# corelab-src/dacapo

Measured on AMD Instinct MI355X. Metric: NTT/s (NTT-equivalents over one run() of the ResNet HEVM program, nt=2^14), higher is better.
Workload: dtype u64; 1 GPU; ResNet-20 (SiLU) HEVM program traced from the reference's examples/benchmarks/ResNet.py with its resnet20.silu.model weights, nt=2^14 slots, N=2^15, 14 x 60-bit primes (SEAL_HEVM.cpp:39-53); one independent ciphertext stream per GPU; streams_per_gpu=1, parallelism=replicas x1 (no collective in the op path)

## Files before the change

dacapo_amd/csrc/batch_ops.hip:

```cpp
#include <stdlib.h>

#include "galois.hpp"
#include "plan.hpp"

namespace dacapo {

constexpr int kBT = 256;

__global__ __launch_bounds__(kBT) void b_tensor_kernel(const MulItem *__restrict__ items, u64 *__restrict__ target, int ell,
                                                        size_t N, const DModulus *__restrict__ mods)
{
    const int i = blockIdx.y, b = blockIdx.z;
    const MulItem it = items[b];
    const DModulus m = mods[i];
    const size_t k = ((size_t)blockIdx.x * kBT + threadIdx.x) * 2;
    const u64x2 a0 = *reinterpret_cast<const u64x2 *>(it.a.limb(0, i, N) + k), a1 = *reinterpret_cast<const u64x2 *>(it.a.limb(1, i, N) + k);
    const u64x2 b0 = *reinterpret_cast<const u64x2 *>(it.b.limb(0, i, N) + k), b1 = *reinterpret_cast<const u64x2 *>(it.b.limb(1, i, N) + k);
    u64x2 c0, c1, c2;
#pragma unroll
    for (int e = 0; e < 2; e++) {
        c0[e] = mulmod(a0[e], b0[e], m);
        Acc128 acc;
        acc.clear();
        acc.mac(a0[e], b1[e]);
// ... 95 lines not shown
        f_dr_lift_fcols(c, acc_last, acc_ps, w.tmp, 2 * B, ell, sp, s);
    } else
        f_dr_icols_lift_fcols(c, acc_last, acc_ps, w.tmp, 2 * B, ell, sp, s);
    last(fused_mac);
}
template <int MODE>
static void b_ks_tail(Context &c, const BatchWs &w, u64 *digits, const KsItem *items, const void *final_items, const u64 *shared_key, int B,
                      int ell, hipStream_t s, const Handoff &h)
{
    b_ks_tail<MODE>(c, w, digits, items, final_items, shared_key, B, ell, s, nullptr, [&](bool fused_mac) {
        f_frows_final(c, (MODE == 1 && fused_mac) ? 4 : MODE, w.tmp, final_items, w.acc, 2 * B, ell, c.K - 1, s, RsItem{}, nullptr, nullptr, h,
                      MODE == 0 && fused_mac);
    });
}

void b_rotate_hops(Context &c, const BatchWs &w, const KsItem *d_items, int B, int ell, hipStream_t s, const Handoff &h, int unique)
{
    if (c.hybrid()) {
        hyb_rotate_hops(c, w, d_items, B, ell, s, unique);
        return;
    }
    f_irows_rot_c1(c, d_items, ell, w.digits, B, s);
    b_ks_tail<0>(c, w, w.digits, d_items, d_items, nullptr, B, ell, s, h);
}

void b_mul_relin(Context &c, const BatchWs &w, const MulItem *d_items, const u64 *relin_key, int B, int ell, hipStream_t s, const Handoff &h)
{
    if (c.hybrid()) {
        hyb_mul_relin(c, w, d_items, relin_key, B, ell, s);
        return;
    }
    const size_t N = c.N;
// ... 419 lines not shown
```

dacapo_amd/csrc/c_api.hip:

```cpp
#include "../../include/dacapo_ckks.h"

#include <stddef.h>
#include <string.h>

#include <algorithm>
#include <vector>

#include "kernels.hpp"
#include "noise_stats.hpp"
#include "plan.hpp"

using namespace dacapo;

#include "c_api_types.hpp"

static inline hipStream_t S(void *s) { return (hipStream_t)s; }
static inline CtView V(const uint64_t *p, long stride) { return CtView{ const_cast<u64 *>(p), stride }; }

namespace {
constexpr int kItemSlots = 64;
constexpr size_t kItemBytes = 128;
static_assert(sizeof(KsItem) <= kItemBytes && sizeof(MulItem) <= kItemBytes && sizeof(RsItem) <= kItemBytes && sizeof(MulRsItem) <= kItemBytes, "item slot too small");
constexpr int kConstSlotWords = 64;
void *item_slot(dc_context *ctx, const void *host_item, size_t bytes, hipStream_t s)
// ... 319 lines not shown
    DC_HIP_CHECK(hipStreamSynchronize(s));
    const char *d = static_cast<const char *>(ctx->mulsum_table);
    b_mul_sum_relin(c, batch_ws(c.ws0), reinterpret_cast<const MulSumItem *>(d), reinterpret_cast<const MulTerm *>(d + kTermsAt), relin_key, 1, ell, s);
    if (alias) launch_ew(c, EwOp::Copy, V(dst, dst_stride), out, out, 2, 2, ell, s);
}
void dc_ct_rotate_hop(dc_context *ctx, uint64_t *dst, long dst_stride, const uint64_t *src, long src_stride,
                      uint32_t galois_elt, const uint64_t *galois_key, int ell, void *stream)
{
    if (overlaps(dst, src)) {
        rotate_hop(*ctx->c, ctx->c->ws0, V(dst, dst_stride), V(src, src_stride), galois_elt, galois_key, ell, S(stream));
        return;
    }
    const KsItem it{ V(src, src_stride), V(dst, dst_stride), galois_key, galois_elt, 0 };
    const KsItem *d = static_cast<const KsItem *>(item_slot(ctx, &it, sizeof(it), S(stream)));
    b_rotate_hops(*ctx->c, batch_ws(ctx->c->ws0), d, 1, ell, S(stream));
}
void dc_ct_rotate_hoisted(dc_context *ctx, uint64_t *const *dsts, long dst_stride, const uint64_t *src, long src_stride,
                          const uint32_t *galois_elts, const uint64_t *const *galois_keys, int count, int ell, void *stream)
{
    const size_t B = (size_t)count;
    const KsItem *d = hoist_items(ctx, "dc_ct_rotate_hoisted", ", where dc_ct_rotate_hop already takes the digits before the automorphism", "hops",
                                  count, ell, B, S(stream), [&](std::vector<KsItem> &h) {
                                      for (size_t b = 0; b < B; b++)
                                          h.push_back(KsItem{ V(src, src_stride), V(dsts[b], dst_stride), galois_keys[b], galois_elts[b], 0 });
                                      h.push_back(KsItem{ V(src, src_stride), V(src, src_stride), nullptr, 1u, 0 });
                                      return (size_t)0;
                                  });
    Context &c = *ctx->c;
    const BatchWs w{ c.ws0.ct_tmp, c.ws0.ks_digits, c.ws0.ks_ext, ctx->hoist_acc, ctx->hoist_tmp };
    hoist_rotate_hops(c, w, d, d + B, count, 1, ell, S(stream));
// ... 124 lines not shown
```

dacapo_amd/csrc/fused_ks.hip:

```cpp
#include "ks_mac.hpp"

namespace dacapo {

struct SrcStrided {
    const u64 *base;
    long stride;
    int prime_base, period;
    __device__ int prime(int z) const { return prime_base + z % period; }
    __device__ u64 load(int z, int g, int) const { return base[(long)z * stride + g]; }
};
template <int E>
__device__ __forceinline__ void rs_operand(u64 (&v)[E], const int (&g)[E], const RsItem &it, const SumSrc *__restrict__ srcs, int p, int i,
                                           size_t N, const DModulus &M)
{
    if (it.count == 0) {
        const u64 *x = it.src.limb(p, i, N);
#pragma unroll
        for (int j = 0; j < E; j++) v[j] = x[g[j]];
    } else {
        u64 s[E];
        Acc128 a[E];
#pragma unroll
        for (int j = 0; j < E; j++) s[j] = 0, a[j].clear();
        int n_plain = 0, n_prod = 0;
// ... 813 lines not shown
    const size_t N = (size_t)1 << logN;
    const DModulus M = mods[pm];
    const u64 *key = MODE == 0 ? items[b].key : shared_key;
    int g[E];
#pragma unroll
    for (int e = 0; e < E; e++) g[e] = tile_gidx<K, LOGE, false>(NP - 1, logN, blockIdx.x, e);
    Acc128 a0[E], a1[E];
#pragma unroll
    for (int e = 0; e < E; e++) a0[e].clear(), a1[e].clear();
    if (MODE == 0 && pmod && m < ell) {
        const KsItem &it = items[b];
        const u64 *c0 = it.src.limb(0, m, N);
        const u64 P = pmod[m];
        u64 cv[E];
        galois_gather<E>(cv, c0, (u32)g[0], it.elt, logN);
#pragma unroll
        for (int e = 0; e < E; e++) a0[e].lo = mulmod(cv[e], P, M);
    }
    if (FOLD && m == ell - 1) {
        const MulRsItem &it = reinterpret_cast<const MulRsItem *>(items)[b];
        const u64 *pa0 = it.a.limb(0, m, N), *pa1 = it.a.limb(1, m, N), *pb0 = it.b.limb(0, m, N), *pb1 = it.b.limb(1, m, N);
        const u64 *pl = it.add ? it.add + (size_t)m * N : nullptr;
        const u64 P = pmod[m];
#pragma unroll
        for (int e = 0; e < E; e++) {
            const u64 va0 = pa0[g[e]], va1 = pa1[g[e]], vb0 = pb0[g[e]], vb1 = pb1[g[e]];
            u64 d0 = mulmod(va0, vb0, M);
            if (pl) d0 = addmod(d0, pl[g[e]], M.q);
            Acc128 t;
            t.clear();
            t.mac(va0, vb1);
            t.mac(va1, vb0);
// ... 430 lines not shown
```

dacapo_amd/csrc/hevm_vm.hip:

```cpp
#include "hevm_vm.hpp"

#include "../../include/dacapo_ckks.h"
#include "c_api_types.hpp"
#include "chacha.hpp"
#include "seal_serial.hpp"

#include <math.h>
#include <string.h>
#include <sys/random.h>

#include <algorithm>
#include <cmath>
#include <chrono>
#include <fstream>
#include <iostream>

namespace dacapo {

constexpr int kVmThreads = 256;

constexpr int kRngCoefs = 8;

__device__ __forceinline__ int rng_cbd(u64 w)
{
// ... 410 lines not shown
                            "switching uses grouped digits, whose lazy sums take no addend\n", ks_flatten, ksp, alpha);
            abort();
        }
        if (!ks_hoist || !ks_lazy) {
            fprintf(stderr, "[dacapo_amd] option ks_flatten_sums = %d needs%s%s%s: a flattened stage is a hoisted lazy sum -- the rotations of one source "
                            "share its decomposition (ks_hoist) and one division by P (ks_lazy_sum)\n", ks_flatten, ks_hoist ? "" : " ks_hoist = 1",
                    !ks_hoist && !ks_lazy ? " and" : "", ks_lazy ? "" : " ks_lazy_sum >= 1");
            abort();
        }
        if (option(OPT_ROT_COMPOSE) != 0) {
            fprintf(stderr, "[dacapo_amd] option ks_flatten_sums = %d does not combine with rot_compose = 1: a memoised hop may serve two rotate "
                            "instructions, and a flattened stage takes its rotations' hops away\n", ks_flatten);
            abort();
        }
    }
    zenc_head = option(OPT_ZENC_HEAD) != 0;
    const int bits = (int)option(OPT_PRIME_BITS);
    ctx.reset(new Context(logN, K, bits, primes, ksp, alpha));
    ctx->ensure_scratch();
    encoder.reset(new HostEncoder(logN));
    use_plan = option(OPT_PLAN) != 0;
    plan_graph = option(OPT_PLAN_GRAPH) != 0;
    plan_dag = option(OPT_PLAN_GRAPH) == 2;
    plan_lanes = option(OPT_PLAN_LANES) >= 2 ? 2 : 1;
    host_encoder = option(OPT_HOST_ENCODER) != 0;
    fold_rescale_into_boot = option(OPT_FOLD_RESCALE_BOOT) != 0;
    lazy_sums = option(OPT_HYB_LAZY_SUM) != 0;
    double_hoist = (lazy_sums && option(OPT_HYB_DOUBLE_HOIST) != 0) || ks_lazy == 2;
    max_batch = std::max(1, (int)option(OPT_MAX_BATCH));
    chain_fusion = option(OPT_CHAIN_FUSION) != 0;
// ... 1637 lines not shown
    case 8: op_mulcc(op.dst, op.lhs, op.rhs); break;
    case 9: op_mulcp(op.dst, op.lhs, op.rhs); break;
    case 10: op_bootstrap(op.dst, op.lhs, op.rhs); break;
    case kOpConj: op_conj(op.dst, op.lhs); break;
    case kOpModRaise: op_modraise(op.dst, op.lhs, op.rhs); break;
    case kOpSetScale: op_setscale(op.dst, op.lhs, op.rhs); break;
    case kOpKeySwitch: op_keyswitch(op.dst, op.lhs, op.rhs); break;
    default: break;
    }
}

void HEVM::execute()
{
    memset(op_counts, 0, sizeof(op_counts));
    n_keyswitch = n_ntt = 0;
    n_hops = n_decomp = 0, n_fold = 0, n_relin_groups = n_relin_products = 0, n_flat_groups = n_flat_members = n_flat_hops = 0;
    t_bootstrap = 0.0;
    int i = (int)((header.hevm_header_size + config.config_body_length) / 8), j = 0;
    for (const WireOp &op : ops) {
        if (debug) {
            std::cout << std::endl;
            std::cout << std::oct << i++ << " " << std::dec << j++ << std::endl;
            std::cout << "opcode [" << op.opcode << "], dst [" << op.dst << "], lhs [" << op.lhs << "], rhs [" << op.rhs << "]"
                      << std::endl;
        }
        if (op.opcode <= 10) op_counts[op.opcode]++;
        if (op.opcode == 0 || (op.opcode > 10 && (op.opcode < kOpConj || op.opcode > kOpKeySwitch))) continue;
        dispatch(op);
    }
    bump_epoch(S());
}
// ... 434 lines not shown
            flat.insert(flat.end(), p.flat_ops.begin(), p.flat_ops.end());
            flat.push_back((int32_t)p.flat_offsets.size());
            flat.insert(flat.end(), p.flat_offsets.begin(), p.flat_offsets.end());
        }
    if (out && cap >= (int64_t)flat.size()) memcpy(out, flat.data(), flat.size() * sizeof(int32_t));
    return (int64_t)flat.size();
}

void hevm_last_run_flatten_stats(void *vm, int64_t *groups, int64_t *members, int64_t *hops_absorbed)
{
    if (groups) *groups = V(vm)->n_flat_groups;
    if (members) *members = V(vm)->n_flat_members;
    if (hops_absorbed) *hops_absorbed = V(vm)->n_flat_hops;
}

int64_t hevm_plan_relin_groups(void *vm, int32_t *out, int64_t cap)
{
    auto h = V(vm);
    if (!h->plan.ready) return -1;
    std::vector<int32_t> flat;
    for (const auto &p : h->plan.pops)
        if (!p.dead && p.kind == HEVM::P_MULSUM) {
            flat.push_back((int32_t)p.ops.size());
            flat.push_back((int32_t)p.op);
            for (size_t k = 0; k < p.ops.size(); k++) flat.push_back((int32_t)p.ops[k]), flat.push_back((int32_t)p.signs[k]);
        }
    if (out && cap >= (int64_t)flat.size()) memcpy(out, flat.data(), flat.size() * sizeof(int32_t));
    return (int64_t)flat.size();
}

// ... 18 lines not shown
```

dacapo_amd/csrc/hevm_vm.hpp:

```cpp
#pragma once
#include "wire_parse.hpp"
#include <algorithm>
#include <complex>
#include <deque>
#include <map>
#include <set>
#include <memory>
#include <string>
#include <unordered_set>
#include <vector>

#include "../../include/hevm_abi.h"
#include "chacha.hpp"
#include "seal_serial.hpp"
#include "kernels.hpp"
#include "encoder.hpp"
#include "io_batch.hpp"
#include "plan.hpp"
#include "plan_flow.hpp"

namespace dacapo {

struct VmAllocs {
    std::unordered_set<void *> live;
// ... 184 lines not shown
        BootItem *d_boot = nullptr;
        RsItem *d_boot_rs = nullptr;
        ZencItem *d_boot_zenc = nullptr;
        size_t zenc_bytes = 0;
        u64 *zenc = nullptr, *boot_ue = nullptr, *boot_tmp = nullptr, *boot_pt[2] = { nullptr, nullptr }, *boot_ptx[2] = { nullptr, nullptr };
        signed char *boot_e = nullptr;
        struct BootChunk { int first, count, target; };
        std::vector<BootChunk> boot_chunks;
        BatchWs ws[2];
        std::vector<hipEvent_t> events;
        std::vector<u64 *> pool;
        int64_t n_keyswitch = 0, n_ntt = 0;
        int64_t n_hops = 0, n_decomp = 0;
        int64_t n_relin_groups = 0, n_relin_products = 0;
        int64_t n_flat_groups = 0, n_flat_members = 0, n_flat_hops = 0;
        int64_t n_fold = 0;
        size_t launches = 0, max_live = 0;
        hipGraph_t graph = nullptr;
        hipGraphExec_t graph_exec = nullptr;
    } plan;
    bool plan_graph = true;
    bool plan_dag = false;
    void capture_plan();
    bool capture_plan_dag();
    void issue_step(const Step &st, hipStream_t q);
    void drop_plan_graph();
    void *plan_alloc(size_t bytes);
    void release_plan();
    void issue_head(hipStream_t s);
    void issue_plan(hipStream_t s);
// ... 16 lines not shown
    void boot_item(CtView src, int src_level, double src_scale, hevm_ctxt &dst, int target_level);
    void plan_zero_encrypt(int first, int B, int t, hipStream_t s);
    void plan_boot_step(int first, int B, int ell, int t, int lane, hipStream_t s, const Handoff &h);
    bool rot_compose = false;
    std::vector<int> compose_rotation(int steps) const;
    mutable std::vector<int> rot_offsets;
    mutable std::set<int> rot_offset_set;
    mutable size_t rot_offsets_epoch = (size_t)-1;
    int boot_secret_weight = 0;
    int secret_weight = 0;
    bool ks_hoist = false;
    int ks_lazy = 0;
    bool ks_fold_rescale = false;
    bool ks_lazy_relin = false;
    int ks_flatten = 0;
    PlanFlow program_flow() const;
    std::vector<FlattenGroup> flatten_groups(const PlanFlow &flow, bool every_key) const;
    bool zenc_head = true;
    static constexpr int kZencChunk = 64;
    int zenc_chunk_hook = 0;
    KsItem *d_hoist_items = nullptr;
    void rotate_hop_vm(CtView dst, CtView src, u32 elt, const u64 *key, int ell);
    bool chain_fusion = true;
    hipStream_t aux_stream = nullptr;
    bool double_hoist = false;
    double *dh_consts = nullptr;
    std::map<int, EncItem> dh_items;
    void ensure_special_limbs(const std::vector<int> &plain_regs);
    bool lazy_sums = false;
    bool fold_rescale_into_boot = false;
    int plan_lanes = 2;
    int plan_level = 1;
    void bump_epoch(hipStream_t s);

    int64_t op_counts[11] = { 0 };
    int64_t n_keyswitch = 0, n_ntt = 0;
    int64_t n_hops = 0, n_decomp = 0;
    int64_t n_fold = 0;
    int64_t n_relin_groups = 0, n_relin_products = 0;
    int64_t n_flat_groups = 0, n_flat_members = 0, n_flat_hops = 0;
    double t_bootstrap = 0.0;

    VmAllocs allocs;
    HEVM() { g_vm_allocs = &allocs; }
    void destroy_device_state();
    size_t key_elems() const { return (size_t)ctx->key_digits() * 2 * ctx->K * ctx->N; }
    void init_context(int logN, int K, const u64 *primes, int dir_ksp = 0, int dir_alpha = 0);
    void generate_keys(const RngKeys &rng, bool secret, bool pub, bool eval);
    void gen_kswitch_key(u64 *key, const u64 *new_key, u64 key_id);
    void gen_kswitch_key_in(Context &c, u64 *key, const u64 *key_sk, const u64 *new_key, u64 key_id);
    void fill_sparse_secret(u64 *dst, int weight, u32 domain);
    void generate_boot_switch_keys();
    size_t swk_down_elems() const { return (size_t)2 * (1 + ctx->ksp) * ctx->N; }
// ... 59 lines not shown
```

dacapo_amd/csrc/options.cpp:

```cpp
#include "options.hpp"

#include "../../include/hevm_abi.h"

#include <stdio.h>
#include <stdlib.h>
#include <string.h>

namespace dacapo {

struct OptDef {
    const char *name;
    long long def;
};
static const OptDef kDefs[OPT_COUNT] = {
    { "logn", 15 },
    { "primes", 14 },
    { "prime_bits", 60 },
    { "ks_special", 1 },
    { "ks_alpha", 0 },
    { "secret_hw", 0 },
    { "boot_secret_hw", 0 },
    { "rot_compose", 0 },
    { "plan", 1 },
    { "plan_graph", 1 },
// ... 2 lines not shown
    { "max_batch", 64 },
    { "plan_level", 1 },
    { "chain_fusion", 1 },
    { "host_encoder", 0 },
    { "online_encode", 0 },
    { "fold_rescale_boot", 0 },
    { "hyb_mfma", 1 },
    { "hyb_fuse", 2 },
    { "hyb_lazy_sum", 0 },
    { "hyb_double_hoist", 0 },
    { "ks_hoist", 0 },
    { "ks_lazy_sum", 0 },
    { "ks_fold_rescale", 0 },
    { "ks_lazy_relin", 0 },
    { "ks_flatten_sums", 0 },
    { "zenc_head", 1 },
    { "seal_compr", 0 },
    { "trace", 0 },
    { "step_profile", 0 },
    { "small_tile_wgs", -1 },
    { "tiny_tile_wgs", 2000 },
    { "wide_tile_wgs", 2048 },
    { "rows_prime_major", 16 },
    { "ntt_full_min_limbs", 768 },
    { "ntt_full_inv_min_limbs", 768 },
    { "ntt_full_persist", -1 },
    { "ntt_full_inv_persist", -1 },
    { "ntt_full_pairs", 1 },
    { "ntt_full_inv_pairs", 1 },
    { "cols_pairs", 1 },
// ... 119 lines not shown
```

dacapo_amd/csrc/options.hpp:

```cpp
#pragma once

namespace dacapo {

enum Opt : int {
    OPT_LOGN,
    OPT_PRIMES,
    OPT_PRIME_BITS,
    OPT_KS_SPECIAL,
    OPT_KS_ALPHA,
    OPT_SECRET_HW,
    OPT_BOOT_SECRET_HW,
    OPT_ROT_COMPOSE,
    OPT_PLAN,
    OPT_PLAN_GRAPH,
    OPT_PLAN_LANES,
    OPT_PLAN_AUX_MIN_COST,
    OPT_MAX_BATCH,
    OPT_PLAN_LEVEL,
    OPT_CHAIN_FUSION,
    OPT_HOST_ENCODER,
    OPT_ONLINE_ENCODE,
    OPT_FOLD_RESCALE_BOOT,
    OPT_HYB_MFMA,
    OPT_HYB_FUSE,
    OPT_HYB_LAZY_SUM,
    OPT_HYB_DOUBLE_HOIST,
    OPT_KS_HOIST,
    OPT_KS_LAZY_SUM,
    OPT_KS_FOLD_RESCALE,
    OPT_KS_LAZY_RELIN,
    OPT_KS_FLATTEN_SUMS,
    OPT_ZENC_HEAD,
    OPT_SEAL_COMPR,
    OPT_TRACE,
    OPT_STEP_PROFILE,
    OPT_SMALL_TILE_WGS,
    OPT_TINY_TILE_WGS,
    OPT_WIDE_TILE_WGS,
    OPT_ROWS_PRIME_MAJOR,
    OPT_NTT_FULL_MIN_LIMBS,
    OPT_NTT_FULL_INV_MIN_LIMBS,
    OPT_NTT_FULL_PERSIST,
    OPT_NTT_FULL_INV_PERSIST,
    OPT_NTT_FULL_PAIRS,
    OPT_NTT_FULL_INV_PAIRS,
    OPT_COLS_PAIRS,
// ... 15 lines not shown
```

dacapo_amd/csrc/plan.hpp:

```cpp
#pragma once
#include "crt_device.hpp"
#include "kernels.hpp"

namespace dacapo {

struct KsItem {
    CtView src, dst;
    const u64 *key;
    u32 elt;
    u32 slot;
    const u64 *plain = nullptr, *plain_sp = nullptr;
};
struct MulItem {
    CtView a, b, dst;
};
struct MulRsItem : MulItem {
    const u64 *add = nullptr;
    const u64 *mul = nullptr;
    long mul_stride = 0;
};
struct MulTerm {
    CtView a, b;
    int sign;
};
struct MulSumItem {
    CtView dst;
// ... 52 lines not shown
    u64 *out = nullptr;
    const CtView *other = nullptr;
    const struct RsItem *rs_items = nullptr;
    const u64 *sk = nullptr;
    const u64 *in = nullptr;
};

struct BatchWs {
    u64 *target = nullptr;
    u64 *digits = nullptr;
    u64 *ext = nullptr;
    u64 *acc = nullptr;
    u64 *tmp = nullptr;
};

void b_rotate_hops(Context &c, const BatchWs &w, const KsItem *d_items, int B, int ell, hipStream_t s, const Handoff &h = Handoff{}, int unique = 0);
void b_mul_relin(Context &c, const BatchWs &w, const MulItem *d_items, const u64 *relin_key, int B, int ell, hipStream_t s,
                 const Handoff &h = Handoff{});
bool mul_relin_rescale_fused(const Context &c, int B, int ell);
void b_mul_relin_rescale(Context &c, const BatchWs &w, const MulRsItem *d_items, const u64 *relin_key, int B, int ell, hipStream_t s,
                         const Handoff &h = Handoff{});
void b_rescale(Context &c, const BatchWs &w, const RsItem *d_items, int B, int ell, hipStream_t s, const SumSrc *d_srcs = nullptr,
               const Handoff &h = Handoff{});
void b_mul_sum_relin(Context &c, const BatchWs &w, const MulSumItem *d_items, const MulTerm *d_terms, const u64 *relin_key, int B, int ell,
                     hipStream_t s);
void hoist_rotate_hops(Context &c, const BatchWs &w, const KsItem *d_items, const KsItem *d_sources, int B, int U, int ell, hipStream_t s);
void hoist_rotate_sum(Context &c, const BatchWs &w, const KsItem *d_items, const KsItem *d_sources, int B, int U, const KsItem *d_groups, int G,
                      int ell, hipStream_t s, bool addend = false);
bool chain_fusion_supported();
void hyb_rotate_hops(Context &c, const BatchWs &w, const KsItem *d_items, int B, int ell, hipStream_t s, int unique = 0);
void hyb_rotate_sum(Context &c, const BatchWs &w, const KsItem *d_items, int B, const KsItem *d_groups, int G, int ell, hipStream_t s, int unique = 0);
// ... 53 lines not shown
```

dacapo_amd/csrc/plan_exec.hip:

```cpp
#include <math.h>
#include <string.h>

#include <algorithm>
#include <chrono>
#include <map>
#include <functional>
#include <queue>
#include <set>
#include <tuple>

#include "hevm_vm.hpp"
#include "plan_flow.hpp"
#include "plan_levels.hpp"

namespace dacapo {

#define ks_ntts(ell) ks_ntt_count(c, (ell))

void *HEVM::plan_alloc(size_t bytes)
{
    void *d = nullptr;
    DC_HIP_CHECK(vm_malloc(&d, bytes));
    plan.owned.push_back(d);
    return d;
// ... 526 lines not shown
                }
            }
        }
    }

    if (double_hoist) {
        std::vector<int> need_sp;
        for (const Pop &p : O)
            if (!p.dead && p.kind == P_ROTSUM)
                for (int pl : p.plains)
                    if (pl >= 0) need_sp.push_back(pl);
        ensure_special_limbs(need_sp);
    }

    int max_wave = 0;
    for (Pop &p : O) {
        if (p.dead) continue;
        int w = 0;
        for (int s : p.srcs) {
            const int dp = V[(size_t)s].def_pop;
            if (dp >= 0) w = std::max(w, O[(size_t)dp].wave);
        }
        p.wave = w + 1;
        max_wave = std::max(max_wave, p.wave);
    }
    int levels_moved = 0;
    if (plan_level == 1) {
        std::vector<int> live, idx(O.size(), -1);
        for (size_t i = 0; i < O.size(); i++)
            if (!O[i].dead) idx[i] = (int)live.size(), live.push_back((int)i);
        const size_t n = live.size();
        std::vector<int> kind(n), level(n), target(n), cap(n), fixed(n), launches(n), link_prev(n, -1), asap(n), first(n + 1, 0), prod, wave(n);
        const bool links = chain_fusion && chain_fusion_supported();
        for (size_t k = 0; k < n; k++) {
            const Pop &p = O[(size_t)live[k]];
            kind[k] = (int)p.kind, level[k] = p.level, target[k] = p.target_level, asap[k] = p.wave;
            cap[k] = (int)step_chunk(p.kind);
            fixed[k] = p.kind == P_ROTSUM;
            launches[k] = kKind[p.kind].launches;
// ... 240 lines not shown
        st.count *= S;
        const size_t B = (size_t)st.count, l = (size_t)st.level;
        switch (st.kind) {
        case P_ROT:
            st.first = (int)h_ks.size();
            {
                const bool hoisted = st.target == -2;
                std::map<const u64 *, u32> slot_of;
                std::vector<KsItem> sources;
                for (int pi : step_pops[s])
                    for (int q = 0; q < S; q++) {
                        const CtView sv = plan_view(O[(size_t)pi].srcs[0], q);
                        if (hoisted && !slot_of.count(sv.p)) sources.push_back(KsItem{ sv, sv, nullptr, 1u, 0 });
                        const u32 slot = (c.hybrid() || hoisted) ? slot_of.emplace(sv.p, (u32)slot_of.size()).first->second : 0u;
                        h_ks.push_back(KsItem{ sv, plan_view(O[(size_t)pi].dst, q), O[(size_t)pi].key, O[(size_t)pi].elt, slot });
                    }
                st.unique = (int)slot_of.size();
                st.gfirst = (int)h_ks.size(), st.gcount = (int)sources.size();
                h_ks.insert(h_ks.end(), sources.begin(), sources.end());
                for (int pi : step_pops[s])
                    if (O[(size_t)pi].rot) P.n_hops += S, P.n_decomp += hoisted ? 0 : S;
                if (hoisted) P.n_decomp += st.unique;
            }
            break;
        case P_ROTSUM: {
            st.first = (int)h_ks.size();
            std::map<const u64 *, u32> slot_of;
            std::vector<KsItem> groups, sources;
            for (int pi : step_pops[s])
                for (int q = 0; q < S; q++) {
// ... 208 lines not shown
        BatchWs &w = P.ws[ln];
        w.target = alloc(need_t), w.digits = alloc(need_d), w.ext = alloc(need_e);
        w.acc = alloc(need_a), w.tmp = alloc(need_m);
    }
    {
        size_t aux_waves = 0;
        for (size_t i = 0; i < P.steps.size(); i++)
            if (P.steps[i].lane == 1 && (i == 0 || P.steps[i - 1].wave != P.steps[i].wave || P.steps[i - 1].lane != 1)) aux_waves++;
        while (P.events.size() < 2 * aux_waves + 2) {
            hipEvent_t e;
            DC_HIP_CHECK(hipEventCreateWithFlags(&e, hipEventDisableTiming));
            P.events.push_back(e);
        }
        if (aux_waves && !aux_stream) DC_HIP_CHECK(hipStreamCreateWithFlags(&aux_stream, hipStreamNonBlocking));
    }
    P.n_keyswitch *= S, P.n_ntt *= S;
    P.ready = true;
    if (plan_graph) capture_plan();
    if (option(OPT_TRACE)) report_plan(sum_stat, max_wave, levels_moved);
}

void HEVM::place_online_encode(const std::vector<std::vector<int>> &step_pops)
{
    Plan &P = plan;
    const std::vector<Pop> &O = P.pops;
    const size_t N = ctx->N;
    std::map<int, std::pair<int, int>> use;
    auto touch = [&](int reg, int w) {
        if (reg < 0) return;
        auto it = use.emplace(reg, std::make_pair(w, w)).first;
        it->second.first = std::min(it->second.first, w), it->second.second = std::max(it->second.second, w);
// ... 200 lines not shown
        size_t multi = 0, launches = 0;
        for (size_t a = 0; a < P.steps.size();) {
            size_t b = a;
            while (b < P.steps.size() && P.steps[b].wave == P.steps[a].wave) b++;
            multi += b - a > 1;
            a = b;
        }
        for (const Step &st : P.steps)
            launches += (size_t)kKind[st.kind].launches;
        fprintf(stderr, "[dacapo_amd] plan levels: plan_level %d moved %d operations: %zu steps in %d waves, %zu waves with more than one step, %zu links, "
                        "%zu step launches (5 per key switch, 3 per rescale, 4 per opcode 10, 1 per limb-wise step, -1 per link), %zu live buffers, "
                        "%zu pool buffers (%.3f GB)\n",
                plan_level, levels_moved, P.steps.size(), max_wave, multi, P.n_fused, launches - P.n_fused, P.max_live, P.pool.size(),
                (double)P.pool.size() * buf_elems * (double)streams * 8 / 1e9);
    }
}

void HEVM::issue_step(const Step &st, hipStream_t q)
{
    Context &c = *ctx;
    Plan &P = plan;
    const BatchWs &w = P.ws[st.lane];
    switch (st.kind) {
    case P_ROT:
        if (st.target == -2) {
            hoist_rotate_hops(c, w, P.d_ks + st.first, P.d_ks + st.gfirst, st.count, st.unique, st.level, q);
            break;
        }
        b_rotate_hops(st.target < 0 ? *bctx : c, w, P.d_ks + st.first, st.count, st.level, q, st.h, st.unique); break;
    case P_ROTSUM:
        if (!c.hybrid()) {
            hoist_rotate_sum(c, w, P.d_ks + st.first, P.d_ks + st.gfirst + st.gcount, st.count, st.unique, P.d_ks + st.gfirst, st.gcount, st.level, q,
                             st.addend);
            break;
        }
        hyb_rotate_sum(c, w, P.d_ks + st.first, st.count, P.d_ks + st.gfirst, st.gcount, st.level, q, st.unique); break;
    case P_MULCC:
        if (st.fold_rs) {
            b_mul_relin_rescale(c, w, P.d_mulrs + st.first, keys.relin, st.count, st.level, q, st.h);
            break;
        }
        b_mul_relin(c, w, P.d_mul + st.first, keys.relin, st.count, st.level, q, st.h); break;
    case P_MULSUM: b_mul_sum_relin(c, w, P.d_mulsum + st.first, P.d_mulsum_terms, keys.relin, st.count, st.level, q); break;
    case P_RESCALE: b_rescale(c, w, P.d_rs + st.first, st.count, st.level, q, P.d_sum_srcs, st.h); break;
// ... 210 lines not shown
}

void HEVM::run_plan()
{
    if (!plan.ready) build_plan();
    Context &c = *ctx;
    Plan &P = plan;
    cur = 0;
    hipStream_t s = S();
    memset(op_counts, 0, sizeof(op_counts));
    for (const WireOp &op : ops)
        if (op.opcode <= 10) op_counts[op.opcode]++;
    n_keyswitch = P.n_keyswitch, n_ntt = P.n_ntt;
    n_hops = P.n_hops, n_decomp = P.n_decomp, n_fold = P.n_fold;
    n_relin_groups = P.n_relin_groups, n_relin_products = P.n_relin_products;
    n_flat_groups = P.n_flat_groups, n_flat_members = P.n_flat_members, n_flat_hops = P.n_flat_hops;
    t_bootstrap = 0.0;
    const long ps = (long)c.K * (long)c.N;
    if (plan_graph) {
        capture_plan();
        if (P.graph_exec)
            DC_HIP_CHECK(hipGraphLaunch(P.graph_exec, s));
        else
            issue_plan(s);
    } else
        issue_plan(s);
    DC_HIP_CHECK(hipStreamSynchronize(s));
    if (P.d_enc_overflow) {
        int overflow = 0;
        DC_HIP_CHECK(hipMemcpy(&overflow, P.d_enc_overflow, sizeof(int), hipMemcpyDeviceToHost));
// ... 19 lines not shown
```

dacapo_amd/lowlevel.py:

```python
from __future__ import annotations

import ctypes as C

import numpy as np

from . import LIB_PATH, LIB_PATH_GW

_lib = None
_libs: dict = {}


def lib_gw():
    return lib(LIB_PATH_GW)


def lib(path=None):
    global _lib
    if path is not None and str(path) != str(LIB_PATH):
        if str(path) not in _libs:
            _libs[str(path)] = _bind(path)
        return _libs[str(path)]
    if _lib is None:
        _lib = _bind(LIB_PATH)
    return _lib
# ... 38 lines not shown
        L.dc_event_elapsed_ms.restype = C.c_float
        L.dc_event_elapsed_ms.argtypes = [vp, vp]
        for f in (L.dc_ntt_forward, L.dc_ntt_inverse):
            f.argtypes = [vp, u64p, lng, i32, vp, i32, i32, vp]
        L.dc_ntt_variant.argtypes = [vp, i32, i32, u64p, lng, i32, vp, i32, i32, vp]
        L.dc_ct_negate.argtypes = [vp, u64p, lng, u64p, lng, i32, vp]
        L.dc_ct_add.argtypes = [vp, u64p, lng, u64p, lng, u64p, lng, i32, vp]
        L.dc_ct_add_plain.argtypes = [vp, u64p, lng, u64p, lng, u64p, i32, vp]
        L.dc_ct_mul_plain.argtypes = [vp, u64p, lng, u64p, lng, u64p, i32, vp]
        L.dc_ct_mul_relin.argtypes = [vp, u64p, lng, u64p, lng, u64p, lng, u64p, i32, vp]
        L.dc_ct_mul_relin_rescale.argtypes = [vp, u64p, lng, u64p, lng, u64p, lng, u64p, u64p, vp, i32, vp]
        L.dc_ct_mul.argtypes = [vp, u64p, lng, u64p, lng, u64p, lng, i32, vp]
        L.dc_ct_relin.argtypes = [vp, u64p, lng, u64p, lng, u64p, i32, vp]
        L.dc_ct_mul_sum_relin.argtypes = [vp, u64p, lng, vp, vp, vp, i32, lng, u64p, i32, vp]
        L.dc_ct_rotate_hop.argtypes = [vp, u64p, lng, u64p, lng, C.c_uint32, u64p, i32, vp]
        L.dc_ct_rotate_hoisted.argtypes = [vp, vp, lng, u64p, lng, vp, vp, i32, i32, vp]
        L.dc_ct_rotate_sum_hoisted.argtypes = [vp, u64p, lng, vp, lng, vp, vp, vp, vp, i32, i32, vp]
        L.dc_ct_rotate_sum_hoisted_add.argtypes = [vp, u64p, lng, u64p, lng, vp, lng, vp, vp, vp, vp, i32, i32, vp]
        L.dc_ct_rescale.argtypes = [vp, u64p, lng, u64p, lng, i32, vp]
        L.dc_ct_modswitch.argtypes = [vp, u64p, lng, u64p, lng, i32, i32, vp]
        L.dc_keyswitch.argtypes = [vp, u64p, lng, u64p, u64p, u64p, u64p, i32, vp]
        L.dc_galois_ntt.argtypes = [vp, u64p, lng, u64p, lng, C.c_uint32, i32, i32, vp]
        L.dc_poly_mul.argtypes = [vp, u64p, u64p, u64p, i32, vp]
        L.dc_poly_add.argtypes = [vp, u64p, u64p, u64p, i32, vp]
        L.dc_poly_error_stats.argtypes = [vp, u64p, lng, u64p, lng, i32, i32, i32, vp, vp]
        L.dc_poly_error_stats.restype = None
        L.dc_galois_elt_from_step.restype = C.c_uint32
        L.dc_galois_elt_from_step.argtypes = [vp, i32]
        from .runner import bind_options

# ... 150 lines not shown
```

dacapo_amd/runner.py:

```python
from __future__ import annotations

import contextlib
import ctypes
import re
import weakref
from pathlib import Path

import numpy as np

from . import LIB_PATH

lw = None


def reinit_lw():
    global lw
    if lw is None:
        lw = bind_vm_lib(LIB_PATH)
    return lw


_vm_libs: dict = {}


# ... 63 lines not shown
    L.hevm_last_run_stats.argtypes = [ctypes.c_void_p, ctypes.POINTER(ctypes.c_int64), ctypes.POINTER(ctypes.c_int64),
                                       ctypes.POINTER(ctypes.c_int64)]
    L.hevm_last_run_hoist_stats.argtypes = [ctypes.c_void_p, ctypes.POINTER(ctypes.c_int64), ctypes.POINTER(ctypes.c_int64)]
    L.hevm_last_run_fold_rescale_stats.argtypes = [ctypes.c_void_p, ctypes.POINTER(ctypes.c_int64)]
    L.hevm_plan_lazy_groups.argtypes = [ctypes.c_void_p, ctypes.POINTER(ctypes.c_int32), ctypes.c_int64]
    L.hevm_plan_lazy_groups.restype = ctypes.c_int64
    L.hevm_plan_relin_groups.argtypes = [ctypes.c_void_p, ctypes.POINTER(ctypes.c_int32), ctypes.c_int64]
    L.hevm_plan_relin_groups.restype = ctypes.c_int64
    L.hevm_last_run_relin_stats.argtypes = [ctypes.c_void_p, ctypes.POINTER(ctypes.c_int64), ctypes.POINTER(ctypes.c_int64)]
    L.hevm_flatten_offsets.argtypes = [ctypes.c_void_p, ctypes.POINTER(ctypes.c_int64), ctypes.c_int]
    L.hevm_flatten_offsets.restype = ctypes.c_int
    L.hevm_plan_flatten_groups.argtypes = [ctypes.c_void_p, ctypes.POINTER(ctypes.c_int32), ctypes.c_int64]
    L.hevm_plan_flatten_groups.restype = ctypes.c_int64
    L.hevm_last_run_flatten_stats.argtypes = [ctypes.c_void_p] + [ctypes.POINTER(ctypes.c_int64)] * 3
    L.hevm_last_run_flatten_stats.restype = None
    L.hevm_set_streams.argtypes = [ctypes.c_void_p, ctypes.c_int]
    L.hevm_select_stream.argtypes = [ctypes.c_void_p, ctypes.c_int]
    L.hevm_encrypt_batch.argtypes = [ctypes.c_void_p, ctypes.c_int64, ctypes.c_void_p, ctypes.c_int, ctypes.c_int64, ctypes.c_int, ctypes.c_int,
                                     ctypes.c_int]
    L.hevm_encrypt_batch.restype = None
    for f in (L.hevm_decrypt_batch, L.hevm_decrypt_result_batch):
        f.argtypes = [ctypes.c_void_p, ctypes.c_int64, ctypes.c_void_p, ctypes.c_int64, ctypes.c_int, ctypes.c_int, ctypes.c_int]
        f.restype = None
    L.hevm_phase_batch.argtypes = [ctypes.c_void_p, ctypes.c_int64, ctypes.c_void_p, ctypes.c_int64, ctypes.c_int, ctypes.c_int]
    L.hevm_phase_batch.restype = ctypes.c_int
    L.hevm_last_io_stats.argtypes = [ctypes.c_void_p, ctypes.POINTER(ctypes.c_int64), ctypes.POINTER(ctypes.c_int64)]
    L.hevm_last_io_stats.restype = None
    L.dc_device_sync.argtypes = []
    L.dc_device_sync.restype = None
    L.hevm_last_run_bootstrap_seconds.argtypes = [ctypes.c_void_p]
# ... 352 lines not shown
    def flatten_stats(self):
        g, m, h = ctypes.c_int64(), ctypes.c_int64(), ctypes.c_int64()
        self.lw.hevm_last_run_flatten_stats(self.vm, ctypes.byref(g), ctypes.byref(m), ctypes.byref(h))
        return {"groups": g.value, "members": m.value, "hops_absorbed": h.value}

    def fold_rescale_stats(self):
        pairs = ctypes.c_int64()
        self.lw.hevm_last_run_fold_rescale_stats(self.vm, ctypes.byref(pairs))
        return pairs.value

    def stats(self):
        counts = (ctypes.c_int64 * 11)()
        ks, ntt = ctypes.c_int64(), ctypes.c_int64()
        self.lw.hevm_last_run_stats(self.vm, counts, ctypes.byref(ks), ctypes.byref(ntt))
        return {"op_counts": list(counts), "keyswitches": ks.value, "ntts": ntt.value,
                "bootstrap_s": float(self.lw.hevm_last_run_bootstrap_seconds(self.vm))}

    def printer(self, latency, rms, mem_usage=0.0):
        bench = re.search(r"optimized/(.*)/(.*)\.(.*)\._", self.hevm_path)
        print("======================================")
        print("---------------Option-----------------")
        if bench:
            print("compiler:", bench.group(1))
            print("benchname:", bench.group(2))
            print("waterline:", bench.group(3))
        print("library:", run_library)
        print("device:", run_hardware)
        print("---------------Result-----------------")
        print("latency:", latency)
        print("rms:", rms)
# ... 3 lines not shown
```

include/dacapo_ckks.h:

```cpp
#ifndef DACAPO_CKKS_H
#define DACAPO_CKKS_H

#include <stddef.h>
#include <stdint.h>

#ifdef __cplusplus
extern "C" {
#endif
#if defined(__GNUC__)
#pragma GCC visibility push(default)
#endif

typedef struct dc_context dc_context;

dc_context *dc_context_create(int logN, int num_primes, int bit_size, const uint64_t *primes);
dc_context *dc_context_create_hybrid(int logN, int num_primes, int special, int alpha);
dc_context *dc_context_create_hybrid_primes(int logN, const uint64_t *primes, int num_primes, int special, int alpha);
int dc_context_key_digits(const dc_context *ctx);
int dc_context_max_level(const dc_context *ctx);
void dc_context_destroy(dc_context *ctx);
int dc_context_logn(const dc_context *ctx);
int dc_context_num_primes(const dc_context *ctx);
void dc_context_primes(const dc_context *ctx, uint64_t *out );
void dc_context_roots(const dc_context *ctx, uint64_t *out );
// ... 31 lines not shown
                     int ell, void *stream);
void dc_ct_mul_relin(dc_context *ctx, uint64_t *dst, long dst_stride, const uint64_t *a, long a_stride, const uint64_t *b,
                     long b_stride, const uint64_t *relin_key, int ell, void *stream);
void dc_ct_mul(dc_context *ctx, uint64_t *dst3, long dst_stride, const uint64_t *a, long a_stride, const uint64_t *b, long b_stride, int ell,
               void *stream);
void dc_ct_relin(dc_context *ctx, uint64_t *dst, long dst_stride, const uint64_t *src3, long src_stride, const uint64_t *relin_key, int ell,
                 void *stream);
#define DC_CT_MUL_SUM_MAX 32
void dc_ct_mul_sum_relin(dc_context *ctx, uint64_t *dst, long dst_stride, const uint64_t *const *as, const uint64_t *const *bs,
                         const int32_t *signs, int count, long src_stride, const uint64_t *relin_key, int ell, void *stream);
void dc_ct_mul_relin_rescale(dc_context *ctx, uint64_t *dst, long dst_stride, const uint64_t *a, long a_stride, const uint64_t *b,
                             long b_stride, const uint64_t *relin_key, const uint64_t *add_plain, const uint64_t *mul_const, int ell,
                             void *stream);
void dc_ct_rotate_hop(dc_context *ctx, uint64_t *dst, long dst_stride, const uint64_t *src, long src_stride,
                      uint32_t galois_elt, const uint64_t *galois_key, int ell, void *stream);
void dc_ct_rotate_hoisted(dc_context *ctx, uint64_t *const *dsts, long dst_stride, const uint64_t *src, long src_stride,
                          const uint32_t *galois_elts, const uint64_t *const *galois_keys, int count, int ell, void *stream);
void dc_ct_rotate_sum_hoisted(dc_context *ctx, uint64_t *dst, long dst_stride, const uint64_t *const *srcs, long src_stride,
                              const uint32_t *galois_elts, const uint64_t *const *galois_keys, const uint64_t *const *plains,
                              const uint64_t *const *plains_sp, int count, int ell, void *stream);
void dc_ct_rotate_sum_hoisted_add(dc_context *ctx, uint64_t *dst, long dst_stride, const uint64_t *addend, long addend_stride,
                                  const uint64_t *const *srcs, long src_stride, const uint32_t *galois_elts,
                                  const uint64_t *const *galois_keys, const uint64_t *const *plains, const uint64_t *const *plains_sp,
                                  int count, int ell, void *stream);
void dc_ct_rescale(dc_context *ctx, uint64_t *dst, long dst_stride, const uint64_t *src, long src_stride, int ell,
                   void *stream);
void dc_ct_modswitch(dc_context *ctx, uint64_t *dst, long dst_stride, const uint64_t *src, long src_stride, int ell, int down,
                     void *stream);

void dc_keyswitch(dc_context *ctx, uint64_t *out, long out_stride, const uint64_t *base0, const uint64_t *base1,
// ... 25 lines not shown
```

include/hevm_abi.h:

```cpp
#ifndef HEVM_ABI_H
#define HEVM_ABI_H

#include <stdbool.h>
#include <stdint.h>

#ifdef __cplusplus
extern "C" {
#endif
#if defined(__GNUC__)
#pragma GCC visibility push(default)
#endif

void *initFullVM(char *dir, bool device);
void *initClientVM(char *dir);
void *initServerVM(char *dir);
void create_context(char *dir);
void load(void *vm, char *constant, char *vmfile);
void loadClient(void *vm, void *is);
void encrypt(void *vm, int64_t i, double *dat, int len);
void decrypt(void *vm, int64_t i, double *dat);
void decrypt_result(void *vm, int64_t i, double *dat);
int64_t getResIdx(void *vm, int64_t i);
void *getCtxt(void *vm, int64_t id);
void preprocess(void *vm);
// ... 22 lines not shown
#endif
void *hevm_context(void *vm);
const uint64_t *hevm_relin_key(void *vm);
const uint64_t *hevm_galois_key(void *vm, uint32_t elt);
const uint64_t *hevm_public_key(void *vm);
int hevm_boot_switch_keys(void *vm, const uint64_t **down, const uint64_t **up, int *down_limbs);
int hevm_key_buffers(void *vm, uint64_t **ptrs, uint64_t *words, int cap);
uint64_t hevm_key_digest(void *vm);
void hevm_keys_replaced(void *vm);
const uint64_t *hevm_plain(void *vm, int64_t i, int32_t *level, double *scale);
const uint64_t *hevm_plain_special(void *vm, int64_t i);
void hevm_load_mem(void *vm, const void *cst, uint64_t cst_len, const void *hevm, uint64_t hevm_len);
void hevm_last_run_stats(void *vm, int64_t *op_counts , int64_t *keyswitches, int64_t *ntts);
void hevm_last_run_hoist_stats(void *vm, int64_t *hops, int64_t *decompositions);
void hevm_last_run_fold_rescale_stats(void *vm, int64_t *pairs);
int64_t hevm_plan_lazy_groups(void *vm, int32_t *out, int64_t cap);
int64_t hevm_plan_relin_groups(void *vm, int32_t *out, int64_t cap);
void hevm_last_run_relin_stats(void *vm, int64_t *groups, int64_t *products);
int hevm_flatten_offsets(void *vm, int64_t *out, int cap);
int64_t hevm_plan_flatten_groups(void *vm, int32_t *out, int64_t cap);
void hevm_last_run_flatten_stats(void *vm, int64_t *groups, int64_t *members, int64_t *hops_absorbed);
void hevm_set_streams(void *vm, int n);
void hevm_select_stream(void *vm, int s);
void hevm_encrypt_batch(void *vm, int64_t arg, const double *vals, int len, int64_t stride, int first_stream, int count, int where);
void hevm_decrypt_batch(void *vm, int64_t reg, double *out, int64_t stride, int first_stream, int count, int where);
void hevm_decrypt_result_batch(void *vm, int64_t i, double *out, int64_t stride, int first_stream, int count, int where);
int hevm_phase_batch(void *vm, int64_t reg, uint64_t *out_dev, int64_t stride, int first_stream, int count);
void hevm_last_io_stats(void *vm, int64_t *launches, int64_t *chunks);
double hevm_last_run_bootstrap_seconds(void *vm);
uint64_t hevm_plaintext_bytes(void *vm);
// ... 28 lines not shown
```

Baseline: 1.442 million NTT/s.

## Fold two-term sums into the preceding rotation hop as an addend

Adds a plan pass that finds a two-ciphertext sum whose one input is a single-use direct rotation and removes the sum. It does this by making the rotation write to the sum's destination and carry the other operand as an addend. The fused key-switch kernel adds the addend (pre-multiplied by P) into the accumulator, which saves a separate elementwise add launch and one ciphertext read/write round trip. The pass then recomputes wave scheduling, which can change how steps are grouped. It is enabled by default only for SEAL-layout contexts with fused MAC below the tile threshold.

```diff
diff --git a/dacapo_amd/csrc/batch_ops.hip b/dacapo_amd/csrc/batch_ops.hip
--- a/dacapo_amd/csrc/batch_ops.hip
+++ b/dacapo_amd/csrc/batch_ops.hip
@@ -133,8 +133,13 @@
     });
 }
 
-void b_rotate_hops(Context &c, const BatchWs &w, const KsItem *d_items, int B, int ell, hipStream_t s, const Handoff &h, int unique)
-{
+void b_rotate_hops(Context &c, const BatchWs &w, const KsItem *d_items, int B, int ell, hipStream_t s, const Handoff &h, int unique, bool addend)
+{
+    if (addend && (c.hybrid() || !fuse_mac() || (long)(c.N >> 10) * B * ell * ell >= fuse_mac_threshold())) {
+        fprintf(stderr, "[dacapo_amd] b_rotate_hops: an item carries an addend, which only the fused middle of SEAL-layout key switching adds "
+                        "(%s)\n", c.hybrid() ? "this context switches keys with grouped digits" : "option ks_fuse_mac = 0, or the batch is above ks_fuse_mac_tiles");
+        abort();
+    }
     if (c.hybrid()) {
         hyb_rotate_hops(c, w, d_items, B, ell, s, unique);
         return;
diff --git a/dacapo_amd/csrc/c_api.hip b/dacapo_amd/csrc/c_api.hip
--- a/dacapo_amd/csrc/c_api.hip
+++ b/dacapo_amd/csrc/c_api.hip
@@ -357,6 +357,19 @@
     const KsItem it{ V(src, src_stride), V(dst, dst_stride), galois_key, galois_elt, 0 };
     const KsItem *d = static_cast<const KsItem *>(item_slot(ctx, &it, sizeof(it), S(stream)));
     b_rotate_hops(*ctx->c, batch_ws(ctx->c->ws0), d, 1, ell, S(stream));
+}
+void dc_ct_rotate_hop_add(dc_context *ctx, uint64_t *dst, long dst_stride, const uint64_t *src, long src_stride, const uint64_t *addend,
+                          long addend_stride, uint32_t galois_elt, const uint64_t *galois_key, int ell, void *stream)
+{
+    if (ctx->c->hybrid()) {
+        fprintf(stderr, "[dacapo_amd] dc_ct_rotate_hop_add: this context switches keys with grouped digits (ks_special > 1); the call is for "
+                        "SEAL-layout keys (use dc_ct_rotate_hop and dc_ct_add)\n");
+        abort();
+    }
+    KsItem it{ V(src, src_stride), V(dst, dst_stride), galois_key, galois_elt, 0 };
+    it.add = V(addend, addend_stride);
+    const KsItem *d = static_cast<const KsItem *>(item_slot(ctx, &it, sizeof(it), S(stream)));
+    b_rotate_hops(*ctx->c, batch_ws(ctx->c->ws0), d, 1, ell, S(stream), Handoff{}, 0, true);
 }
 void dc_ct_rotate_hoisted(dc_context *ctx, uint64_t *const *dsts, long dst_stride, const uint64_t *src, long src_stride,
                           const uint32_t *galois_elts, const uint64_t *const *galois_keys, int count, int ell, void *stream)
diff --git a/dacapo_amd/csrc/fused_ks.hip b/dacapo_amd/csrc/fused_ks.hip
--- a/dacapo_amd/csrc/fused_ks.hip
+++ b/dacapo_amd/csrc/fused_ks.hip
@@ -851,8 +851,18 @@
         const u64 P = pmod[m];
         u64 cv[E];
         galois_gather<E>(cv, c0, (u32)g[0], it.elt, logN);
-#pragma unroll
-        for (int e = 0; e < E; e++) a0[e].lo = mulmod(cv[e], P, M);
+        if (it.add.p) {
+            const u64 *y0 = it.add.limb(0, m, N) + g[0], *y1 = it.add.limb(1, m, N) + g[0];
+#pragma unroll
+            for (int e = 0; e < E; e += 2) {
+                const u64x2 v0 = *reinterpret_cast<const u64x2 *>(y0 + e), v1 = *reinterpret_cast<const u64x2 *>(y1 + e);
+                a0[e].lo = mulmod(addmod(cv[e], v0.x, M.q), P, M), a0[e + 1].lo = mulmod(addmod(cv[e + 1], v0.y, M.q), P, M);
+                a1[e].lo = mulmod(v1.x, P, M), a1[e + 1].lo = mulmod(v1.y, P, M);
+            }
+        } else {
+#pragma unroll
+            for (int e = 0; e < E; e++) a0[e].lo = mulmod(cv[e], P, M);
+        }
     }
     if (FOLD && m == ell - 1) {
         const MulRsItem &it = reinterpret_cast<const MulRsItem *>(items)[b];
diff --git a/dacapo_amd/csrc/hevm_vm.hip b/dacapo_amd/csrc/hevm_vm.hip
--- a/dacapo_amd/csrc/hevm_vm.hip
+++ b/dacapo_amd/csrc/hevm_vm.hip
@@ -448,6 +448,7 @@
             abort();
         }
     }
+    ks_fold_add = option(OPT_KS_FOLD_ADD) != 0;
     zenc_head = option(OPT_ZENC_HEAD) != 0;
     const int bits = (int)option(OPT_PRIME_BITS);
     ctx.reset(new Context(logN, K, bits, primes, ksp, alpha));
@@ -2115,7 +2116,7 @@
 {
     memset(op_counts, 0, sizeof(op_counts));
     n_keyswitch = n_ntt = 0;
-    n_hops = n_decomp = 0, n_fold = 0, n_relin_groups = n_relin_products = 0, n_flat_groups = n_flat_members = n_flat_hops = 0;
+    n_hops = n_decomp = 0, n_fold = 0, n_add_folds = 0, n_relin_groups = n_relin_products = 0, n_flat_groups = n_flat_members = n_flat_hops = 0;
     t_bootstrap = 0.0;
     int i = (int)((header.hevm_header_size + config.config_body_length) / 8), j = 0;
     for (const WireOp &op : ops) {
@@ -2580,6 +2581,8 @@
     if (hops_absorbed) *hops_absorbed = V(vm)->n_flat_hops;
 }
 
+int64_t hevm_last_run_add_fold_stats(void *vm) { return V(vm)->n_add_folds; }
+
 int64_t hevm_plan_relin_groups(void *vm, int32_t *out, int64_t cap)
 {
     auto h = V(vm);
diff --git a/dacapo_amd/csrc/hevm_vm.hpp b/dacapo_amd/csrc/hevm_vm.hpp
--- a/dacapo_amd/csrc/hevm_vm.hpp
+++ b/dacapo_amd/csrc/hevm_vm.hpp
@@ -222,6 +222,7 @@
         int64_t n_hops = 0, n_decomp = 0;
         int64_t n_relin_groups = 0, n_relin_products = 0;
         int64_t n_flat_groups = 0, n_flat_members = 0, n_flat_hops = 0;
+        int64_t n_add_folds = 0;
         int64_t n_fold = 0;
         size_t launches = 0, max_live = 0;
         hipGraph_t graph = nullptr;
@@ -268,6 +269,7 @@
     bool ks_fold_rescale = false;
     bool ks_lazy_relin = false;
     int ks_flatten = 0;
+    bool ks_fold_add = true;
     PlanFlow program_flow() const;
     std::vector<FlattenGroup> flatten_groups(const PlanFlow &flow, bool every_key) const;
     bool zenc_head = true;
@@ -291,6 +293,7 @@
     int64_t n_keyswitch = 0, n_ntt = 0;
     int64_t n_hops = 0, n_decomp = 0;
     int64_t n_fold = 0;
+    int64_t n_add_folds = 0;
     int64_t n_relin_groups = 0, n_relin_products = 0;
     int64_t n_flat_groups = 0, n_flat_members = 0, n_flat_hops = 0;
     double t_bootstrap = 0.0;
diff --git a/dacapo_amd/csrc/options.cpp b/dacapo_amd/csrc/options.cpp
--- a/dacapo_amd/csrc/options.cpp
+++ b/dacapo_amd/csrc/options.cpp
@@ -40,6 +40,7 @@
     { "ks_fold_rescale", 0 },
     { "ks_lazy_relin", 0 },
     { "ks_flatten_sums", 0 },
+    { "ks_fold_add", 1 },
     { "zenc_head", 1 },
     { "seal_compr", 0 },
     { "trace", 0 },
diff --git a/dacapo_amd/csrc/options.hpp b/dacapo_amd/csrc/options.hpp
--- a/dacapo_amd/csrc/options.hpp
+++ b/dacapo_amd/csrc/options.hpp
@@ -30,6 +30,7 @@
     OPT_KS_FOLD_RESCALE,
     OPT_KS_LAZY_RELIN,
     OPT_KS_FLATTEN_SUMS,
+    OPT_KS_FOLD_ADD,
     OPT_ZENC_HEAD,
     OPT_SEAL_COMPR,
     OPT_TRACE,
diff --git a/dacapo_amd/csrc/plan.hpp b/dacapo_amd/csrc/plan.hpp
--- a/dacapo_amd/csrc/plan.hpp
+++ b/dacapo_amd/csrc/plan.hpp
@@ -10,6 +10,7 @@
     u32 elt;
     u32 slot;
     const u64 *plain = nullptr, *plain_sp = nullptr;
+    CtView add = CtView{ nullptr, 0 };
 };
 struct MulItem {
     CtView a, b, dst;
@@ -92,7 +93,8 @@
     u64 *tmp = nullptr;
 };
 
-void b_rotate_hops(Context &c, const BatchWs &w, const KsItem *d_items, int B, int ell, hipStream_t s, const Handoff &h = Handoff{}, int unique = 0);
+void b_rotate_hops(Context &c, const BatchWs &w, const KsItem *d_items, int B, int ell, hipStream_t s, const Handoff &h = Handoff{}, int unique = 0,
+                   bool addend = false);
 void b_mul_relin(Context &c, const BatchWs &w, const MulItem *d_items, const u64 *relin_key, int B, int ell, hipStream_t s,
                  const Handoff &h = Handoff{});
 bool mul_relin_rescale_fused(const Context &c, int B, int ell);
diff --git a/dacapo_amd/csrc/plan_exec.hip b/dacapo_amd/csrc/plan_exec.hip
--- a/dacapo_amd/csrc/plan_exec.hip
+++ b/dacapo_amd/csrc/plan_exec.hip
@@ -564,15 +564,50 @@
     }
 
     int max_wave = 0;
-    for (Pop &p : O) {
-        if (p.dead) continue;
-        int w = 0;
-        for (int s : p.srcs) {
-            const int dp = V[(size_t)s].def_pop;
-            if (dp >= 0) w = std::max(w, O[(size_t)dp].wave);
-        }
-        p.wave = w + 1;
-        max_wave = std::max(max_wave, p.wave);
+    auto asap_waves = [&]() {
+        max_wave = 0;
+        for (Pop &p : O) {
+            if (p.dead) continue;
+            int w = 0;
+            for (int s : p.srcs) {
+                const int dp = V[(size_t)s].def_pop;
+                if (dp >= 0) w = std::max(w, O[(size_t)dp].wave);
+            }
+            p.wave = w + 1;
+            max_wave = std::max(max_wave, p.wave);
+        }
+    };
+    asap_waves();
+    if (ks_fold_add && !c.hybrid() && option(OPT_KS_FUSE_MAC) != 0) {
+        std::vector<int> asap(O.size(), 0);
+        for (size_t i = 0; i < O.size(); i++) asap[i] = O[i].wave;
+        std::set<int> folded;
+        for (size_t si = 0; si < O.size(); si++) {
+            Pop &s = O[si];
+            if (s.dead || s.kind != P_SUM || s.srcs.size() != 2) continue;
+            if (std::any_of(s.src_plain.begin(), s.src_plain.end(), [](int pl) { return pl >= 0; })) continue;
+            if ((long long)(N >> 10) * (long long)step_chunk(P_ROT) * S * s.level * s.level >= option(OPT_KS_FUSE_MAC_TILES)) continue;
+            for (size_t w = 0; w < 2; w++) {
+                const int hv = s.srcs[w], a = s.srcs[1 - w], hi = own_pop(hv);
+                if (hi < 0 || a == hv) continue;
+                Pop &h = O[(size_t)hi];
+                if (h.kind != P_ROT || h.rot != 1 || h.target_level != 0 || !h.direct || h.op < 0 || h.addend >= 0 || h.level != s.level) continue;
+                if (V[(size_t)hv].uses != 1 || V[(size_t)hv].pinned || V[(size_t)s.dst].root != s.dst) continue;
+                const int ar = V[(size_t)a].root, ap = V[(size_t)ar].def_pop;
+                const int aw = ap < 0 ? 0 : folded.count(ar) ? asap[(size_t)ap] + 1 : asap[(size_t)ap];
+                if (ap >= 0 && (ap >= hi || O[(size_t)ap].dead || aw >= asap[(size_t)hi])) continue;
+                h.dst = s.dst, h.addend = a, h.srcs.push_back(a);
+                V[(size_t)s.dst].def_pop = hi;
+                V[(size_t)hv].uses = 0, V[(size_t)hv].def_pop = -1;
+                s.dead = true;
+                folded.insert(s.dst);
+                P.n_add_folds++;
+                break;
+            }
+        }
+        for (Val &v : V)
+            if (folded.count(v.root)) v.def_pop = V[(size_t)v.root].def_pop;
+        if (P.n_add_folds) asap_waves();
     }
     int levels_moved = 0;
     if (plan_level == 1) {
@@ -843,6 +878,7 @@
                         if (hoisted && !slot_of.count(sv.p)) sources.push_back(KsItem{ sv, sv, nullptr, 1u, 0 });
                         const u32 slot = (c.hybrid() || hoisted) ? slot_of.emplace(sv.p, (u32)slot_of.size()).first->second : 0u;
                         h_ks.push_back(KsItem{ sv, plan_view(O[(size_t)pi].dst, q), O[(size_t)pi].key, O[(size_t)pi].elt, slot });
+                        if (O[(size_t)pi].addend >= 0) h_ks.back().add = plan_view(O[(size_t)pi].addend, q), st.addend = true;
                     }
                 st.unique = (int)slot_of.size();
                 st.gfirst = (int)h_ks.size(), st.gcount = (int)sources.size();
@@ -1081,7 +1117,7 @@
         }
         if (aux_waves && !aux_stream) DC_HIP_CHECK(hipStreamCreateWithFlags(&aux_stream, hipStreamNonBlocking));
     }
-    P.n_keyswitch *= S, P.n_ntt *= S;
+    P.n_keyswitch *= S, P.n_ntt *= S, P.n_add_folds *= S;
     P.ready = true;
     if (plan_graph) capture_plan();
     if (option(OPT_TRACE)) report_plan(sum_stat, max_wave, levels_moved);
@@ -1312,6 +1348,9 @@
                 plan_level, levels_moved, P.steps.size(), max_wave, multi, P.n_fused, launches - P.n_fused, P.max_live, P.pool.size(),
                 (double)P.pool.size() * buf_elems * (double)streams * 8 / 1e9);
     }
+    if (P.n_add_folds)
+        fprintf(stderr, "[dacapo_amd] plan folds: %lld two-term sums ride on their rotation's last hop as its addend (option ks_fold_add)\n",
+                (long long)P.n_add_folds);
 }
 
 void HEVM::issue_step(const Step &st, hipStream_t q)
@@ -1325,7 +1364,7 @@
             hoist_rotate_hops(c, w, P.d_ks + st.first, P.d_ks + st.gfirst, st.count, st.unique, st.level, q);
             break;
         }
-        b_rotate_hops(st.target < 0 ? *bctx : c, w, P.d_ks + st.first, st.count, st.level, q, st.h, st.unique); break;
+        b_rotate_hops(st.target < 0 ? *bctx : c, w, P.d_ks + st.first, st.count, st.level, q, st.h, st.unique, st.addend); break;
     case P_ROTSUM:
         if (!c.hybrid()) {
             hoist_rotate_sum(c, w, P.d_ks + st.first, P.d_ks + st.gfirst + st.gcount, st.count, st.unique, P.d_ks + st.gfirst, st.gcount, st.level, q,
@@ -1566,6 +1605,7 @@
     n_keyswitch = P.n_keyswitch, n_ntt = P.n_ntt;
     n_hops = P.n_hops, n_decomp = P.n_decomp, n_fold = P.n_fold;
     n_relin_groups = P.n_relin_groups, n_relin_products = P.n_relin_products;
+    n_add_folds = P.n_add_folds;
     n_flat_groups = P.n_flat_groups, n_flat_members = P.n_flat_members, n_flat_hops = P.n_flat_hops;
     t_bootstrap = 0.0;
     const long ps = (long)c.K * (long)c.N;
diff --git a/dacapo_amd/lowlevel.py b/dacapo_amd/lowlevel.py
--- a/dacapo_amd/lowlevel.py
+++ b/dacapo_amd/lowlevel.py
@@ -76,6 +76,7 @@
         L.dc_ct_relin.argtypes = [vp, u64p, lng, u64p, lng, u64p, i32, vp]
         L.dc_ct_mul_sum_relin.argtypes = [vp, u64p, lng, vp, vp, vp, i32, lng, u64p, i32, vp]
         L.dc_ct_rotate_hop.argtypes = [vp, u64p, lng, u64p, lng, C.c_uint32, u64p, i32, vp]
+        L.dc_ct_rotate_hop_add.argtypes = [vp, u64p, lng, u64p, lng, u64p, lng, C.c_uint32, u64p, i32, vp]
         L.dc_ct_rotate_hoisted.argtypes = [vp, vp, lng, u64p, lng, vp, vp, i32, i32, vp]
         L.dc_ct_rotate_sum_hoisted.argtypes = [vp, u64p, lng, vp, lng, vp, vp, vp, vp, i32, i32, vp]
         L.dc_ct_rotate_sum_hoisted_add.argtypes = [vp, u64p, lng, u64p, lng, vp, lng, vp, vp, vp, vp, i32, i32, vp]
diff --git a/dacapo_amd/runner.py b/dacapo_amd/runner.py
--- a/dacapo_amd/runner.py
+++ b/dacapo_amd/runner.py
@@ -101,6 +101,8 @@
     L.hevm_plan_flatten_groups.restype = ctypes.c_int64
     L.hevm_last_run_flatten_stats.argtypes = [ctypes.c_void_p] + [ctypes.POINTER(ctypes.c_int64)] * 3
     L.hevm_last_run_flatten_stats.restype = None
+    L.hevm_last_run_add_fold_stats.argtypes = [ctypes.c_void_p]
+    L.hevm_last_run_add_fold_stats.restype = ctypes.c_int64
     L.hevm_set_streams.argtypes = [ctypes.c_void_p, ctypes.c_int]
     L.hevm_select_stream.argtypes = [ctypes.c_void_p, ctypes.c_int]
     L.hevm_encrypt_batch.argtypes = [ctypes.c_void_p, ctypes.c_int64, ctypes.c_void_p, ctypes.c_int, ctypes.c_int64, ctypes.c_int, ctypes.c_int,
@@ -483,6 +485,7 @@
         ks, ntt = ctypes.c_int64(), ctypes.c_int64()
         self.lw.hevm_last_run_stats(self.vm, counts, ctypes.byref(ks), ctypes.byref(ntt))
         return {"op_counts": list(counts), "keyswitches": ks.value, "ntts": ntt.value,
+                "add_folds": int(self.lw.hevm_last_run_add_fold_stats(self.vm)),
                 "bootstrap_s": float(self.lw.hevm_last_run_bootstrap_seconds(self.vm))}
 
     def printer(self, latency, rms, mem_usage=0.0):
diff --git a/include/dacapo_ckks.h b/include/dacapo_ckks.h
--- a/include/dacapo_ckks.h
+++ b/include/dacapo_ckks.h
@@ -69,6 +69,8 @@
                              void *stream);
 void dc_ct_rotate_hop(dc_context *ctx, uint64_t *dst, long dst_stride, const uint64_t *src, long src_stride,
                       uint32_t galois_elt, const uint64_t *galois_key, int ell, void *stream);
+void dc_ct_rotate_hop_add(dc_context *ctx, uint64_t *dst, long dst_stride, const uint64_t *src, long src_stride, const uint64_t *addend,
+                          long addend_stride, uint32_t galois_elt, const uint64_t *galois_key, int ell, void *stream);
 void dc_ct_rotate_hoisted(dc_context *ctx, uint64_t *const *dsts, long dst_stride, const uint64_t *src, long src_stride,
                           const uint32_t *galois_elts, const uint64_t *const *galois_keys, int count, int ell, void *stream);
 void dc_ct_rotate_sum_hoisted(dc_context *ctx, uint64_t *dst, long dst_stride, const uint64_t *const *srcs, long src_stride,
diff --git a/include/hevm_abi.h b/include/hevm_abi.h
--- a/include/hevm_abi.h
+++ b/include/hevm_abi.h
@@ -60,6 +60,7 @@
 void hevm_last_run_stats(void *vm, int64_t *op_counts , int64_t *keyswitches, int64_t *ntts);
 void hevm_last_run_hoist_stats(void *vm, int64_t *hops, int64_t *decompositions);
 void hevm_last_run_fold_rescale_stats(void *vm, int64_t *pairs);
+int64_t hevm_last_run_add_fold_stats(void *vm);
 int64_t hevm_plan_lazy_groups(void *vm, int32_t *out, int64_t cap);
 int64_t hevm_plan_relin_groups(void *vm, int32_t *out, int64_t cap);
 void hevm_last_run_relin_stats(void *vm, int64_t *groups, int64_t *products);
```

Measured after the change: 1.482 million NTT/s (median of 6 runs). +2.8%, better.
